# neggles/neurosis

Hardware: AMD Instinct MI355X
Metric: train images/sec (node) SDXL 1024^2 (higher is better)
Workload: dtype bf16

## Files before the change

include/neurosis_hip.h:

```cpp
#ifndef NEUROSIS_HIP_H
#define NEUROSIS_HIP_H

#ifdef __cplusplus
extern "C" {
#endif

const char* nk_last_error(void);
int nk_abi_version(void);

int nk_linear_fwd(const void* x, const void* w, const float* bias, const void* residual, void* y,
                  int M, int N, int K, long ldx, long ldw, long ldr, long ldy, float alpha, void* stream);
int nk_linear_dgrad(const void* dy, const void* w, const void* dx_add, void* dx, int M, int N, int K,
                    long lddy, long ldw, long ldadd, long lddx, void* stream);
long nk_linear_fwd_geglu_ok(int M, int I, int K);
int nk_linear_fwd_geglu(const void* x, const void* w, const float* bias, void* u, void* h, int M, int I, int K, long ldx, long ldw, long ldu,
                        long ldh, void* stream);
int nk_linear_dgrad_geglu(const void* dy, const void* w, const void* u, void* du, int M, int N, int I, long lddy, long ldw, long ldu,
                          long lddu, void* stream);
int nk_linear_fwd_geglu_s(const void* x, const void* w, const float* bias, void* s, void* h, int M, int I, int K, long ldx, long ldw, long lds,
                          long ldh, void* stream);
int nk_linear_dgrad_geglu_s(const void* dy, const void* w, const void* s, void* du, int M, int N, int I, long lddy, long ldw, long lds,
                            long lddu, void* stream);
int nk_linear_wgrad(const void* dy, const void* x, float* dw, int M, int N, int K, long lddy, long ldx,
                    long lddw, int accumulate, void* stream);
int nk_linear_wgrad_bias(const void* dy, const void* x, float* dw, float* dbias, int M, int N, int K, long lddy, long ldx, long lddw,
                         int accumulate, void* stream);

int nk_gemm_sk_status(void);

int nk_health_status(void);
int nk_health_clear(void);
int nk_health_export(int* dst, void* stream);
int nk_health_import(const int* src, void* stream);
int nk_debug_raise_health(void* stream);
int nk_debug_stamp(unsigned long long* dst, void* stream);
int nk_debug_launch_log(int mode);
long nk_debug_launch_names(char* buf, long cap);

int nk_colsum_batched(const void* dy, float* out, float* ws, long M, int N, long ld, int nbatch, int accumulate, void* stream);

int nk_linear_fwd_batched(const void* const* x, const void* const* w, void* const* y, int count, int M, int N, int K,
                          long ldx, long ldw, long ldy, void* stream);

int nk_linear_wgrad_batched(const void* const* dy, const void* const* x, float* const* dw, float* const* dbias, int count, int M, int N,
                            int K, long lddy, long ldx, long lddw, int accumulate, void* stream);

typedef struct NkConvDesc {
  int N, H, W, Cin;
  int Cout, KH, KW;
  int stride;
  int pad_t, pad_l;
  int Ho, Wo;
  int upsample;
} NkConvDesc;
int nk_conv2d_fwd(const NkConvDesc* d, const void* x, const void* w, const float* bias, const void* rowvec,
                  const void* residual, void* y, void* stream);
long nk_conv2d_stats_tiles(const NkConvDesc* d, int stats_groups);
int nk_conv2d_fwd_stats(const NkConvDesc* d, const void* x, const void* w, const float* bias, const void* rowvec, const void* residual,
                        void* y, float* stats_part, int stats_groups, void* stream);
int nk_conv3x3_few_channels_fwd(const void* x, const void* w, const float* bias, void* y, int N, int H, int W, int Cout, int cin_real,
                                void* stream);
int nk_conv_weight_flip(const void* w, void* wt, int Cout, int Cin, int taps, void* stream);
long nk_conv2d_dgrad_flipped_ok(const NkConvDesc* d);
int nk_conv2d_dgrad_flipped(const NkConvDesc* d, const void* dy, const void* wt, void* dx, void* stream);
int nk_conv2d_dgrad(const NkConvDesc* d, const void* dy, const void* w, void* dx, void* stream);
int nk_conv2d_wgrad(const NkConvDesc* d, const void* dy, const void* x, float* dw, int accumulate, void* stream);
int nk_conv2d_wgrad_bias(const NkConvDesc* d, const void* dy, const void* x, float* dw, float* dbias, int accumulate, void* stream);

typedef struct NkAttnDesc {
  int B, H, Lq, Lk, D;
  long sq, sk, sv, so;
  long bq, bk, bv, bo;
  long sdq, sdk, sdv, sdo;
  long bdq, bdk, bdv, bdo;
  float scale;
  int causal;
} NkAttnDesc;
int nk_attention_fwd(const NkAttnDesc* d, const void* q, const void* k, const void* v, void* o, float* lse,
                     void* stream);
long nk_attention_bwd_ws_floats(const NkAttnDesc* d);
int nk_attention_bwd(const NkAttnDesc* d, const void* q, const void* k, const void* v, const void* o,
                     const float* lse, const void* d_o, void* dq, void* dk, void* dv, float* delta_ws, void* stream);
int nk_attention_bwd_causal(const NkAttnDesc* d, const void* q, const void* k, const void* v, const void* o,
                            const float* lse, const void* d_o, void* dq, void* dk, void* dv, void* stream);
int nk_attention_relbias_fwd(const NkAttnDesc* d, const void* q, const void* k, const void* v, void* o, const float* rel, void* stream);
int nk_attention_relbias_fwd_lse(const NkAttnDesc* d, const void* q, const void* k, const void* v, void* o, float* lse, const float* rel, void* stream);
long nk_attention_relbias_bwd_ws_floats(const NkAttnDesc* d);
int nk_attention_relbias_bwd(const NkAttnDesc* d, const void* q, const void* k, const void* v, const void* o, const float* lse, const void* d_o, void* dq,
                             void* dk, void* dv, const float* rel, float* d_rel, float* ws, int accumulate, void* stream);
int nk_relbias_bucket_sum(const float* d_rel, const int* buckets, float* d_weight, int H, int L, int num_buckets, int accumulate, void* stream);
int nk_softmax_rows(void* s, long M, int L, void* stream);

long nk_groupnorm_ws_floats(int N, int HW, int C, int G);
int nk_groupnorm_fwd(const void* x, const float* gamma, const float* beta, void* y, float* mean, float* rstd,
                     float* ws, int N, int HW, int C, int G, float eps, int silu, void* stream);
int nk_groupnorm_sums(const void* x, float* sums, float* ws, int N, int HW, int C, int G, void* stream);
long nk_groupnorm_sums_ws_floats(int N, int nparts, int G);
int nk_groupnorm_sums_from_parts(const float* part, float* sums, float* ws, int N, int nparts, int G, void* stream);
int nk_groupnorm_apply(const void* x, const float* sums, const float* gamma, const float* beta, void* y, float* mean, float* rstd,
                       int N, int HW, int C, int G, float eps, int silu, void* stream);
int nk_groupnorm_bwd(const void* dy, const void* x, const float* gamma, const float* beta, const float* mean,
                     const float* rstd, const void* dx_add, void* dx, float* dgamma, float* dbeta, float* ws,
                     int N, int HW, int C, int G, int silu, int accumulate, void* stream);
int nk_groupnorm_mod_fwd(const void* x, const float* gamma, const float* beta, const void* mod, void* y, float* mean, float* rstd,
                         float* ws, int N, int HW, int C, int G, float eps, int silu, void* stream);
int nk_groupnorm_mod_apply(const void* x, const float* sums, const float* gamma, const float* beta, const void* mod, void* y, float* mean,
                           float* rstd, int N, int HW, int C, int G, float eps, int silu, void* stream);
int nk_groupnorm_mod_bwd(const void* dy, const void* x, const float* gamma, const float* beta, const void* mod, const float* mean,
                         const float* rstd, const void* dx_add, void* dx, float* dgamma, float* dbeta, void* dmod, float* ws,
                         int N, int HW, int C, int G, int silu, int accumulate, void* stream);

int nk_layernorm_fwd(const void* x, const float* gamma, const float* beta, void* y, float* mean, float* rstd,
                     int M, int C, float eps, void* stream);
long nk_layernorm_ws_floats(int M, int C);
int nk_rmsnorm_fwd(const void* x, const float* gamma, void* y, int M, int C, float eps, void* stream);
int nk_rmsnorm_fwd_rstd(const void* x, const float* gamma, void* y, float* rstd, int M, int C, float eps, void* stream);
long nk_rmsnorm_bwd_ws_floats(int M, int C);
int nk_rmsnorm_bwd(const void* dy, const void* x, const float* gamma, const float* rstd, const void* dx_add, void* dx, float* dgamma, float* ws, int M, int C,
                   int accumulate, void* stream);
int nk_layernorm_bwd(const void* dy, const void* x, const float* gamma, const float* mean, const float* rstd,
// ... 189 lines not shown
```

neurosis_amd/csrc/elementwise.hip:

```cpp
#include "../../include/neurosis_hip.h"
#include "nk_common.h"
#include "nk_ew.h"
#include "nk_reduce.h"
#include "norm_plan.h"

struct GegluFwd {
  const bf16_t* u; bf16_t* y; int I;
  __device__ void operator()(long, long row, int ch) const {
    float a[8], g[8];
    ew_load(u + row * 2 * I + ch * 8, a);
    ew_load(u + row * 2 * I + I + ch * 8, g);
#pragma unroll
    for (int e = 0; e < 8; ++e) a[e] *= gelu_erf(g[e]);
    ew_store(y + row * I + ch * 8, a);
  }
};
struct GegluBwd {
  const bf16_t *dy, *u; bf16_t* du; int I;
  __device__ void operator()(long, long row, int ch) const {
    float a[8], g[8], d[8], da[8], dg[8];
    ew_load(u + row * 2 * I + ch * 8, a);
    ew_load(u + row * 2 * I + I + ch * 8, g);
    ew_load(dy + row * I + ch * 8, d);
#pragma unroll
// ... 415 lines not shown
    if (p < HW && c < Cpad) dst[((long)n * HW + p) * Cpad + c] = f2bf(tile[tx][j]);
  }
}
template <typename DstT>
__global__ void nhwc_to_nchw_kernel(const bf16_t* __restrict__ src, DstT* __restrict__ dst, int C, int HW, int Cpad) {
  __shared__ float tile[32][33];
  const int n = blockIdx.z;
  const int p0 = blockIdx.x * 32, c0 = blockIdx.y * 32;
  const int tx = threadIdx.x & 31, ty = threadIdx.x >> 5;
  for (int j = ty; j < 32; j += 8) {
    int p = p0 + j, c = c0 + tx;
    tile[j][tx] = (p < HW && c < C) ? bf2f(src[((long)n * HW + p) * Cpad + c]) : 0.f;
  }
  __syncthreads();
  for (int j = ty; j < 32; j += 8) {
    int c = c0 + j, p = p0 + tx;
    if (c < C && p < HW) {
      float v = tile[tx][j];
      if constexpr (sizeof(DstT) == 4) dst[((long)n * C + c) * HW + p] = v;
      else dst[((long)n * C + c) * HW + p] = f2bf(v);
    }
  }
}
__global__ __launch_bounds__(256) void conv_weight_flip_kernel(const bf16_t* __restrict__ w, bf16_t* __restrict__ wt, int Cout, int Cin, int taps) {
  __shared__ bf16_t tile[64][64 + 8];
  const int tap = blockIdx.z, co0 = blockIdx.y * 64, ci0 = blockIdx.x * 64;
  const int tid = threadIdx.x;
#pragma unroll
  for (int it = 0; it < 2; ++it) {
    const int idx = tid + 256 * it;
    const int r = idx >> 3, ch = idx & 7;
    uint4_t v = {0u, 0u, 0u, 0u};
    if (co0 + r < Cout && ci0 + ch * 8 < Cin) v = *(const uint4_t*)(w + ((long)(co0 + r) * taps + tap) * Cin + ci0 + ch * 8);
    const bf16_t* e = (const bf16_t*)&v;
#pragma unroll
    for (int k = 0; k < 8; ++k) tile[ch * 8 + k][r] = e[k];
  }
  __syncthreads();
  const int tflip = taps - 1 - tap;
#pragma unroll
  for (int it = 0; it < 2; ++it) {
    const int idx = tid + 256 * it;
    const int r = idx >> 3, ch = idx & 7;
    if (ci0 + r < Cin && co0 + ch * 8 < Cout)
      *(uint4_t*)(wt + ((long)(ci0 + r) * taps + tflip) * Cout + co0 + ch * 8) = *(const uint4_t*)&tile[r][ch * 8];
  }
}
extern "C" int nk_conv_weight_flip(const void* w, void* wt, int Cout, int Cin, int taps, void* stream) {
  NK_CHECK_ARG(w && wt && Cout > 0 && Cin > 0 && taps > 0 && taps <= 65535);
  NK_CHECK_ARG((Cout & 7) == 0 && (Cin & 7) == 0);
  hipLaunchKernelGGL(conv_weight_flip_kernel, dim3((Cin + 63) / 64, (Cout + 63) / 64, taps), dim3(256), 0, (hipStream_t)stream, (const bf16_t*)w, (bf16_t*)wt,
                     Cout, Cin, taps);
  return nk_check_launch("conv_weight_flip_kernel");
}

__global__ __launch_bounds__(256) void conv3x3_few_channels_kernel(const bf16_t* __restrict__ x, const bf16_t* __restrict__ w, const float* __restrict__ bias,
                                                                   bf16_t* __restrict__ y, int N, int H, int W, int Cout, int groups_per_wave) {
  const int lane = threadIdx.x & 63, wave = threadIdx.x >> 6;
  const int r = lane & 15, g = lane >> 4;
  const int co_base = blockIdx.y * 128;
  bf16x8_t wf[8][2];
#pragma unroll
  for (int b = 0; b < 8; ++b) {
    const int co = co_base + b * 16 + r;
    uint2_t t0 = {0u, 0u}, t1 = {0u, 0u}, t8 = {0u, 0u};
    if (co < Cout) {
      t0 = *(const uint2_t*)(w + ((long)co * 9 + 2 * g) * 8);
      t1 = *(const uint2_t*)(w + ((long)co * 9 + 2 * g + 1) * 8);
      if (g == 0) t8 = *(const uint2_t*)(w + ((long)co * 9 + 8) * 8);
    }
    wf[b][0] = __builtin_bit_cast(bf16x8_t, (uint4_t){t0.x, t0.y, t1.x, t1.y});
    wf[b][1] = __builtin_bit_cast(bf16x8_t, (uint4_t){t8.x, t8.y, 0u, 0u});
  }
  const int nloc = (g & 1) * 16 + (g >> 1) * 8;
  float bv[4][8];
#pragma unroll
  for (int h = 0; h < 4; ++h)
#pragma unroll
    for (int e = 0; e < 8; ++e) {
      const int co = co_base + h * 32 + nloc + e;
      bv[h][e] = (bias && co < Cout) ? bias[co] : 0.f;
    }
  const long total = (long)N * H * W;
  const long gw = (long)blockIdx.x * 4 + wave;
  const int HW = H * W;
  const int ta = 2 * g, tb = 2 * g + 1;
  const int dya = ta / 3 - 1, dxa = ta % 3 - 1, dyb = tb / 3 - 1, dxb = tb % 3 - 1;

  auto fetch = [&](long grp, uint2_t& a, uint2_t& b, uint2_t& c) {
    a = (uint2_t){0u, 0u}; b = a; c = a;
    const long pix = grp * 16 + r;
    if (pix >= total) return;
    const int n = (int)(pix / HW);
    const int rem = (int)(pix - (long)n * HW);
    const int py = rem / W, px = rem - py * W;
    const bf16_t* img = x + (long)n * HW * 8;
    int yy = py + dya, xx = px + dxa;
    if ((unsigned)yy < (unsigned)H && (unsigned)xx < (unsigned)W) a = *(const uint2_t*)(img + ((long)yy * W + xx) * 8);
    yy = py + dyb; xx = px + dxb;
    if ((unsigned)yy < (unsigned)H && (unsigned)xx < (unsigned)W) b = *(const uint2_t*)(img + ((long)yy * W + xx) * 8);
    if (g == 0) {
      yy = py + 1; xx = px + 1;
      if (yy < H && xx < W) c = *(const uint2_t*)(img + ((long)yy * W + xx) * 8);
    }
  };

// ... 470 lines not shown
```

neurosis_amd/csrc/ops_gemm.hip:

```cpp
#include "../../include/neurosis_hip.h"
#include "nk_gemm.h"
#include <string.h>

static NkGemmParams zero_params() {
  NkGemmParams p;
  memset(&p, 0, sizeof(p));
  p.alpha = 1.0f;
  p.fRowsPerBatch = make_fastdiv(1);
  p.ga.fWo = p.ga.fHoWo = p.ga.fC = p.ga.fKW = make_fastdiv(1);
  p.gb.fWo = p.gb.fHoWo = p.gb.fC = p.gb.fKW = make_fastdiv(1);
  p.tw.fCout = make_fastdiv(1);
  return p;
}

extern "C" int nk_linear_fwd(const void* x, const void* w, const float* bias, const void* residual, void* y,
                             int M, int N, int K, long ldx, long ldw, long ldr, long ldy, float alpha,
                             void* stream) {
  NkGemmParams p = zero_params();
  p.A = (const bf16_t*)x; p.lda = ldx;
  p.B = (const bf16_t*)w; p.ldb = ldw;
  p.M = M; p.N = N; p.K = K;
  p.C = y; p.ldc = ldy;
  p.bias = bias;
  p.residual = (const bf16_t*)residual; p.ldr = ldr;
// ... 208 lines not shown
  g.div = d->stride; g.need_even = d->stride - 1;
  g.fWo = make_fastdiv(Win); g.fHoWo = make_fastdiv(Hin * Win);
  g.fC = make_fastdiv(d->Cout); g.fKW = make_fastdiv(d->KW);
  p.A = (const bf16_t*)dy; p.ga = g;
  p.B = (const bf16_t*)w;
  p.tw.co_stride = (long)d->KH * d->KW * d->Cin;
  p.tw.tap_stride = d->Cin;
  p.tw.fCout = make_fastdiv(d->Cout);
  p.M = d->N * Hin * Win; p.N = d->Cin; p.K = d->KH * d->KW * d->Cout;
  p.C = dx; p.ldc = d->Cin;
  return nk_gemm_dispatch(p, NK_OP_KCG, NK_OP_MCT, 0, 0, (hipStream_t)stream);
}

extern "C" long nk_conv2d_dgrad_flipped_ok(const NkConvDesc* d) {
  if (check_conv(d) || d->KH != 3 || d->KW != 3 || d->stride != 1 || d->pad_t != 1 || d->pad_l != 1) return 0;
  const int Hin = d->upsample ? 2 * d->H : d->H, Win = d->upsample ? 2 * d->W : d->W;
  if (d->Ho != Hin || d->Wo != Win) return 0;
  NkConvDesc t = *d;
  t.H = Hin; t.W = Win; t.Cin = d->Cout; t.Cout = d->Cin; t.upsample = 0;
  NkGemmParams p = conv_fwd_params(&t, nullptr, nullptr, nullptr, nullptr, nullptr, nullptr);
  return nk_halo_tiles_per_image(p, nullptr) > 0;
}

extern "C" int nk_conv2d_dgrad_flipped(const NkConvDesc* d, const void* dy, const void* wt, void* dx, void* stream) {
  NK_CHECK_ARG(nk_conv2d_dgrad_flipped_ok(d) == 1);
  const int Hin = d->upsample ? 2 * d->H : d->H, Win = d->upsample ? 2 * d->W : d->W;
  NkConvDesc t = *d;
  t.H = Hin; t.W = Win; t.Cin = d->Cout; t.Cout = d->Cin; t.upsample = 0;
  NkGemmParams p = conv_fwd_params(&t, dy, wt, nullptr, nullptr, nullptr, dx);
  return nk_gemm_dispatch(p, NK_OP_KCG, NK_OP_KC, 0, 0, (hipStream_t)stream);
}

static int conv_wgrad(const NkConvDesc* d, const void* dy, const void* x, float* dw, float* dbias, int accumulate, void* stream) {
  if (int e = check_conv(d)) return e;
  NkGemmParams p = zero_params();
  p.A = (const bf16_t*)dy; p.lda = d->Cout;
  p.B = (const bf16_t*)x; p.gb = fwd_gather(d);
  p.M = d->Cout; p.N = d->KH * d->KW * d->Cin; p.K = d->N * d->Ho * d->Wo;
  p.C = dw; p.ldc = p.N;
  p.accumulate = accumulate;
  p.dbias = dbias;
  p.halo_nb = (d->KH == 3 && d->KW == 3) ? d->N : 0;
  return nk_gemm_dispatch(p, NK_OP_MC, NK_OP_MCG, 1, 1, (hipStream_t)stream);
}
extern "C" int nk_conv2d_wgrad(const NkConvDesc* d, const void* dy, const void* x, float* dw, int accumulate,
                               void* stream) {
  return conv_wgrad(d, dy, x, dw, nullptr, accumulate, stream);
}
extern "C" int nk_conv2d_wgrad_bias(const NkConvDesc* d, const void* dy, const void* x, float* dw, float* dbias, int accumulate,
                                    void* stream) {
  NK_CHECK_ARG(dbias != nullptr);
  return conv_wgrad(d, dy, x, dw, dbias, accumulate, stream);
}
```

neurosis_amd/lib.py:

```python
from __future__ import annotations

import ctypes as C
import os
from pathlib import Path

import torch

CSRC = Path(__file__).resolve().parent / "csrc"
LIB_PATH = CSRC / "libneurosis_hip.so"

vp, i32, i64, f32 = C.c_void_p, C.c_int, C.c_long, C.c_float


class NkConvDesc(C.Structure):
    _fields_ = [(n, i32) for n in ("N", "H", "W", "Cin", "Cout", "KH", "KW", "stride", "pad_t", "pad_l", "Ho", "Wo", "upsample")]


class NkAttnDesc(C.Structure):
    _fields_ = (
        [(n, i32) for n in ("B", "H", "Lq", "Lk", "D")]
        + [(n, i64) for n in ("sq", "sk", "sv", "so", "bq", "bk", "bv", "bo", "sdq", "sdk", "sdv", "sdo", "bdq", "bdk", "bdv", "bdo")]
        + [("scale", f32), ("causal", i32)]
    )


NK_COLPART_MAX = 32


class NkColpartBatch(C.Structure):
    _fields_ = [("part", vp * NK_COLPART_MAX), ("dgamma", vp * NK_COLPART_MAX), ("dbeta", vp * NK_COLPART_MAX), ("nrows", i32 * NK_COLPART_MAX),
                ("C", i32 * NK_COLPART_MAX), ("accumulate", i32 * NK_COLPART_MAX), ("n", i32)]


cdp, adp = C.POINTER(NkConvDesc), C.POINTER(NkAttnDesc)

SIGNATURES: dict[str, list] = {
    "nk_linear_fwd": [vp, vp, vp, vp, vp, i32, i32, i32, i64, i64, i64, i64, f32, vp],
    "nk_linear_dgrad": [vp, vp, vp, vp, i32, i32, i32, i64, i64, i64, i64, vp],
    "nk_linear_dgrad_geglu": [vp, vp, vp, vp, i32, i32, i32, i64, i64, i64, i64, vp],
    "nk_linear_fwd_geglu": [vp, vp, vp, vp, vp, i32, i32, i32, i64, i64, i64, i64, vp],
    "nk_linear_fwd_geglu_s": [vp, vp, vp, vp, vp, i32, i32, i32, i64, i64, i64, i64, vp],
    "nk_linear_dgrad_geglu_s": [vp, vp, vp, vp, i32, i32, i32, i64, i64, i64, i64, vp],
    "nk_linear_wgrad": [vp, vp, vp, i32, i32, i32, i64, i64, i64, i32, vp],
    "nk_linear_fwd_batched": [C.POINTER(vp), C.POINTER(vp), C.POINTER(vp), i32, i32, i32, i32, i64, i64, i64, vp],
    "nk_linear_wgrad_batched": [C.POINTER(vp), C.POINTER(vp), C.POINTER(vp), C.POINTER(vp), i32, i32, i32, i32, i64, i64, i64, i32, vp],
    "nk_linear_wgrad_bias": [vp, vp, vp, vp, i32, i32, i32, i64, i64, i64, i32, vp],
    "nk_conv2d_wgrad_bias": [cdp, vp, vp, vp, vp, i32, vp],
    "nk_conv2d_fwd": [cdp, vp, vp, vp, vp, vp, vp, vp],
    "nk_conv2d_fwd_stats": [cdp, vp, vp, vp, vp, vp, vp, vp, i32, vp],
    "nk_conv_weight_flip": [vp, vp, i32, i32, i32, vp],
    "nk_conv3x3_few_channels_fwd": [vp, vp, vp, vp, i32, i32, i32, i32, i32, vp],
    "nk_conv2d_dgrad": [cdp, vp, vp, vp, vp],
    "nk_conv2d_dgrad_flipped": [cdp, vp, vp, vp, vp],
    "nk_conv2d_wgrad": [cdp, vp, vp, vp, i32, vp],
    "nk_attention_fwd": [adp, vp, vp, vp, vp, vp, vp],
    "nk_attention_bwd": [adp, vp, vp, vp, vp, vp, vp, vp, vp, vp, vp, vp],
    "nk_attention_bwd_causal": [adp, vp, vp, vp, vp, vp, vp, vp, vp, vp, vp],
    "nk_attention_relbias_fwd": [adp, vp, vp, vp, vp, vp, vp],
    "nk_attention_relbias_fwd_lse": [adp, vp, vp, vp, vp, vp, vp, vp],
    "nk_attention_relbias_bwd": [adp, vp, vp, vp, vp, vp, vp, vp, vp, vp, vp, vp, vp, i32, vp],
    "nk_relbias_bucket_sum": [vp, vp, vp, i32, i32, i32, i32, vp],
    "nk_softmax_rows": [vp, i64, i32, vp],
    "nk_softmax_rows_bwd": [vp, vp, i64, i32, f32, vp],
    "nk_groupnorm_fwd": [vp, vp, vp, vp, vp, vp, vp, i32, i32, i32, i32, f32, i32, vp],
    "nk_groupnorm_sums": [vp, vp, vp, i32, i32, i32, i32, vp],
    "nk_groupnorm_sums_from_parts": [vp, vp, vp, i32, i32, i32, vp],
    "nk_groupnorm_apply": [vp, vp, vp, vp, vp, vp, vp, i32, i32, i32, i32, f32, i32, vp],
    "nk_groupnorm_bwd": [vp, vp, vp, vp, vp, vp, vp, vp, vp, vp, vp, i32, i32, i32, i32, i32, i32, vp],
    "nk_groupnorm_mod_fwd": [vp, vp, vp, vp, vp, vp, vp, vp, i32, i32, i32, i32, f32, i32, vp],
    "nk_groupnorm_mod_apply": [vp, vp, vp, vp, vp, vp, vp, vp, i32, i32, i32, i32, f32, i32, vp],
    "nk_groupnorm_mod_bwd": [vp, vp, vp, vp, vp, vp, vp, vp, vp, vp, vp, vp, vp, i32, i32, i32, i32, i32, i32, vp],
    "nk_layernorm_fwd": [vp, vp, vp, vp, vp, vp, i32, i32, f32, vp],
    "nk_rmsnorm_fwd": [vp, vp, vp, i32, i32, f32, vp],
    "nk_rmsnorm_fwd_rstd": [vp, vp, vp, vp, i32, i32, f32, vp],
    "nk_rmsnorm_bwd": [vp, vp, vp, vp, vp, vp, vp, vp, i32, i32, i32, vp],
    "nk_layernorm_bwd": [vp, vp, vp, vp, vp, vp, vp, vp, vp, vp, i32, i32, i32, vp],
    "nk_layernorm_bwd_dx": [vp, vp, vp, vp, vp, vp, vp, i32, i32, vp],
    "nk_layernorm_bwd_rows": [vp, vp, vp, vp, vp, vp, vp, vp, i32, i32, vp],
    "nk_colpart_reduce_batch": [C.POINTER(NkColpartBatch), vp],
    "nk_layernorm_bwd_params": [vp, vp, vp, vp, vp, vp, vp, i32, i32, i32, vp],
    "nk_geglu_fwd": [vp, vp, i64, i32, vp],
    "nk_geglu_bwd": [vp, vp, vp, i64, i32, vp],
    "nk_geglu_fwd_s": [vp, vp, vp, i64, i32, vp],
    "nk_geglu_bwd_s": [vp, vp, vp, i64, i32, vp],
    "nk_silu_fwd": [vp, vp, i64, vp],
    "nk_gelu_fwd": [vp, vp, i64, i32, vp],
    "nk_gated_gelu_tanh_fwd": [vp, vp, i64, i32, vp],
    "nk_gelu_bwd": [vp, vp, vp, i64, i32, vp],
    "nk_act_bwd": [vp, vp, vp, i64, i32, vp],
    "nk_gated_gelu_tanh_bwd": [vp, vp, vp, i64, i32, vp],
    "nk_embedding_bwd": [vp, vp, i64, vp, vp, i32, i32, i32, i32, i32, i32, vp],
    "nk_gather_rows_bwd": [vp, i64, vp, vp, i32, i32, i32, vp],
    "nk_wgrad_few_rows": [vp, i64, vp, i64, vp, i64, i32, i32, i32, i32, vp],
    "nk_vq_search": [vp, i64, vp, vp, vp, i64, i32, i32, vp],
    "nk_vq_code_stats": [vp, vp, i64, vp, vp, i64, i32, i32, vp],
    "nk_vq_quantize": [vp, vp, vp, i64, vp, vp, vp, i64, i32, i32, i32, vp],
    "nk_gumbel_logits": [vp, i64, vp, vp, vp, i64, i64, i32, i32, vp],
    "nk_gumbel_noise": [vp, i64, i32, vp, i32, vp],
    "nk_gumbel_softmax_fwd": [vp, i64, vp, vp, i32, f32, vp, vp, vp, vp, i64, i32, vp],
    "nk_gumbel_softmax_bwd": [vp, i64, vp, vp, f32, f32, i64, i32, vp],
    "nk_resample_planes": [vp, vp, vp, vp, vp, vp, i32, vp, vp, vp, i32, i64, i32, i32, i32, i32, vp],
    "nk_vit_patchify": [vp, vp, vp, i32, i32, i32, i32, vp],
    "nk_vit_patchify_bwd": [vp, vp, vp, vp, i32, i32, i32, i32, i32, vp],
    "nk_vit_tokens": [vp, vp, vp, vp, i32, i32, i32, vp],
    "nk_vit_tokens_bwd": [vp, vp, i32, i32, i32, vp],
    "nk_vit_add_ln": [vp, vp, vp, vp, vp, i32, vp, vp, vp, i32, i32, f32, vp],
    "nk_vit_cls_head_fwd": [vp, i64, vp, vp, vp, vp, vp, vp, vp, i32, i32, i32, f32, vp],
# ... 4 lines not shown
    "nk_leaky_relu_bwd": [vp, vp, vp, i64, f32, vp],
    "nk_maxpool2x2_fwd": [vp, vp, i32, i32, i32, i32, vp],
    "nk_maxpool2x2_bwd": [vp, vp, vp, i32, i32, i32, i32, vp],
    "nk_maxpool_fwd": [vp, vp, i32, i32, i32, i32, i32, i32, vp],
    "nk_maxpool_bwd": [vp, vp, vp, i32, i32, i32, i32, i32, i32, vp],
    "nk_lpips_layer_fwd": [vp, vp, vp, vp, vp, i32, i32, i32, f32, i32, vp],
    "nk_lpips_layer_bwd": [vp, vp, vp, vp, vp, i32, i32, i32, f32, vp],
    "nk_batchnorm_fwd": [vp, vp, vp, vp, vp, vp, vp, vp, vp, i64, i32, f32, f32, f32, vp],
    "nk_batchnorm_bwd": [vp, vp, vp, vp, vp, vp, vp, vp, vp, vp, i64, i32, f32, i32, vp],
    "nk_batchnorm_eval": [vp, vp, vp, vp, vp, vp, vp, i64, i32, f32, f32, vp],
    "nk_silu_bwd": [vp, vp, vp, i64, vp],
    "nk_add": [vp, vp, vp, i64, vp],
    "nk_dropout": [vp, vp, vp, i64, i32, i64, i64, i64, vp, i32, i32, f32, vp],
    "nk_dropout_draw": [vp, vp, vp],
    "nk_cat_channels": [vp, vp, vp, i64, i32, i32, vp],
    "nk_split_channels": [vp, vp, vp, i64, i32, i32, vp],
    "nk_upsample2x_bwd": [vp, vp, i32, i32, i32, i32, vp],
    "nk_upsample2x_fwd": [vp, vp, i32, i32, i32, i32, vp],
    "nk_avgpool2x_fwd": [vp, vp, i32, i32, i32, i32, vp],
    "nk_avgpool2x_bwd": [vp, vp, i32, i32, i32, i32, vp],
    "nk_nchw_to_nhwc": [vp, i32, vp, i32, i32, i32, i32, f32, vp],
    "nk_nhwc_to_nchw": [vp, vp, i32, i32, i32, i32, i32, vp],
    "nk_cast_f32_to_bf16": [vp, vp, i64, vp],
    "nk_cast_bf16_to_f32": [vp, vp, i64, vp],
    "nk_colsum": [vp, vp, vp, i64, i32, i64, i32, vp],
    "nk_colsum_batched": [vp, vp, vp, i64, i32, i64, i32, i32, vp],
    "nk_timestep_embedding": [vp, vp, i32, i32, f32, vp],
    "nk_edm_prepare": [vp, vp, vp, vp, vp, vp, i32, i32, i32, i32, vp],
    "nk_edm_prepare_cat": [vp, vp, vp, vp, vp, vp, vp, i32, i32, i32, i32, i32, vp],
    "nk_edm_loss": [vp, vp, vp, vp, vp, vp, vp, vp, i32, i32, i32, i32, f32, vp],
    "nk_sample_prepare": [vp, vp, vp, i32, i32, i32, i32, i32, vp],
    "nk_sample_prepare_cat": [vp, vp, vp, vp, vp, i32, i32, i32, i32, i32, i32, vp],
    "nk_sample_denoise": [vp, vp, vp, vp, f32, vp, i32, i32, i32, i32, i32, vp],
    "nk_sample_euler_step": [vp, vp, vp, vp, vp, vp, f32, vp, vp, i32, i32, i32, i32, i32, vp],
    "nk_adamw_flat": [vp, vp, vp, vp, vp, i64, f32, f32, f32, f32, f32, i32, f32, vp],
    "nk_ema_flat": [vp, vp, i64, f32, vp],
    "nk_debug_raise_health": [vp],
    "nk_debug_stamp": [vp, vp],
    "nk_debug_launch_log": [i32],
    "nk_health_clear": [],
    "nk_health_export": [vp, vp],
    "nk_health_import": [vp, vp],
    "nk_adafactor_init": [vp, vp],
    "nk_adafactor_chunk": [vp, vp],
    "nk_came_chunk": [vp, vp],
    "nk_adamw8bit_step": [vp, vp],
}

SIZE_QUERIES: dict[str, list] = {
    "nk_groupnorm_ws_floats": [i32, i32, i32, i32],
    "nk_groupnorm_sums_ws_floats": [i32, i32, i32],
    "nk_conv2d_stats_tiles": [cdp, i32],
    "nk_conv2d_dgrad_flipped_ok": [cdp],
    "nk_linear_fwd_geglu_ok": [i32, i32, i32],
    "nk_layernorm_ws_floats": [i32, i32],
    "nk_layernorm_part_rows": [i32],
    "nk_colsum_ws_floats": [i64, i32],
    "nk_batchnorm_ws_floats": [i64, i32],
    "nk_lpips_layer_ws_floats": [i32, i32],
    "nk_attention_bwd_ws_floats": [adp],
    "nk_attention_relbias_bwd_ws_floats": [adp],
    "nk_rmsnorm_bwd_ws_floats": [i32, i32],
    "nk_vq_search_ws_floats": [i64, i32],
    "nk_vq_quantize_ws_floats": [i64],
    "nk_gumbel_softmax_ws_floats": [i64],
    "nk_resample_ws_floats": [i64, i32, i32, i32, i32],
    "nk_adafactor_tensor_bytes": [],
    "nk_came_tensor_bytes": [],
    "nk_adamw8bit_tensor_bytes": [],
    "nk_gemm_sk_status": [],
    "nk_health_status": [],
    "nk_debug_launch_names": [C.c_char_p, i64],
}

_lib = None


class NkError(RuntimeError):
    pass


def load() -> C.CDLL:
    global _lib
    if _lib is not None:
        return _lib
    path = Path(os.environ.get("NEUROSIS_HIP_LIB", LIB_PATH))
    if not path.exists():
        raise NkError(
            f"{path} not found: the HIP extension is not built. Run `python -c 'import __graft_entry__ as g; g.build()'` "
            "(or `make -C neurosis_amd/csrc`). There is no CPU fallback for the product path."
        )
    lib = C.CDLL(str(path))
    lib.nk_last_error.restype = C.c_char_p
    lib.nk_last_error.argtypes = []
    lib.nk_abi_version.restype = i32
    lib.nk_abi_version.argtypes = []
    for name, argtypes in SIGNATURES.items():
        fn = getattr(lib, name)
        fn.argtypes = argtypes
        fn.restype = i32
    for name, argtypes in SIZE_QUERIES.items():
        fn = getattr(lib, name)
        fn.argtypes = argtypes
        fn.restype = i64
    _lib = lib
    return lib
# ... 24 lines not shown
```

neurosis_amd/ops.py:

```python
from __future__ import annotations

import ctypes as C
import math
import os
import threading
import weakref
from dataclasses import dataclass
from typing import Callable, Optional

import torch
from torch import Tensor

from . import lib
from .lib import NkAttnDesc, NkConvDesc, call, query

BF16 = torch.bfloat16


class EngineState:

    _live = weakref.WeakSet()

    def __init__(self, wgrad_stream=None):
        self.grad_accumulate = False
# ... 424 lines not shown
            call("nk_geglu_fwd_s", u.data_ptr(), h.data_ptr(), u.data_ptr(), M, I, _stream())
        else:
            h = geglu_fwd(u)[0]
    return u, h, _linear_bwd(x if x_saved is None else x_saved, weight, bias, True)


def _linear_bwd(x_in, weight: Tensor, bias: Optional[Tensor], need_dx: bool):
    def bwd(dy: Tensor, dx_add: Optional[Tensor] = None, geglu_u: Optional[Tensor] = None, geglu_s: Optional[Tensor] = None):
        entry = "nk_linear_dgrad_geglu"
        if geglu_s is not None:
            if geglu_u is not None:
                raise ValueError("linear bwd: geglu_u and geglu_s are exclusive")
            geglu_u, entry = geglu_s, "nk_linear_dgrad_geglu_s"
        x = x_in() if callable(x_in) else x_in
        queued = _wgrad_queue is not None and _wgrad_queue.takes(weight) and dy.is_contiguous() and x.is_contiguous()
        db = grad_flat(bias) if bias is not None else None
        if queued:
            _wgrad_queue.add(dy, x, g2d(weight), db)
        else:
            on_wgrad_stream(lambda: gemm_tn_f32(dy, x, g2d(weight), wgrad_mode(weight), dbias=db), dy, x, owner=weight)
        if not need_dx:
            return None
        if geglu_u is not None:
            if dx_add is not None:
                raise ValueError("linear bwd: geglu_u and dx_add are exclusive")
            M, N = dy.shape
            K = weight.shape[1]
            _check2d(geglu_u, "geglu_u")
            if geglu_u.shape != (M, 2 * K):
                raise ValueError(f"linear bwd: geglu_u must be [{M}, {2 * K}], got {tuple(geglu_u.shape)}")
            du = torch.empty(M, 2 * K, dtype=BF16, device=dy.device)
            wq = w2d(weight)
            call(entry, dy.data_ptr(), wq.data_ptr(), geglu_u.data_ptr(), du.data_ptr(), M, N, K, dy.stride(0), wq.stride(0),
                 geglu_u.stride(0), du.stride(0), _stream())
            return du
        return gemm_nn(dy, w2d(weight), dx_add)

    return bwd


def _conv_desc(N, H, W, Cin, Cout, KH, KW, stride, pad_t, pad_l, Ho, Wo, upsample) -> NkConvDesc:
    return NkConvDesc(N, H, W, Cin, Cout, KH, KW, stride, pad_t, pad_l, Ho, Wo, int(upsample))


def groupnorm_sums(x: Img, groups: int) -> Tensor:
    if x.sums is not None and x.sums.shape == (x.N, 2 * groups):
        return x.sums
    sums = torch.empty(x.N, 2 * groups, dtype=torch.float32, device=x.t.device)
    ws = _ws(query("nk_groupnorm_ws_floats", x.N, x.H * x.W, x.C, groups), x.t.device)
    call("nk_groupnorm_sums", x.t.data_ptr(), sums.data_ptr(), ws.data_ptr(), x.N, x.H * x.W, x.C, groups, _stream())
    return sums


def conv2d_fwd(x: Img, weight: Tensor, bias: Optional[Tensor], stride: int = 1, padding=1, upsample: bool = False,
               rowvec: Optional[Tensor] = None, residual: Optional[Tensor] = None, need_dx: bool = True,
               asym_pad: bool = False, stats_groups: Optional[int] = None, cin_real: Optional[int] = None):
    Cout, Cin, KH, KW = weight.shape
    if x.C != Cin:
        raise ValueError(f"conv2d: input has {x.C} channels, weight expects {Cin}")
    Hin, Win = (2 * x.H, 2 * x.W) if upsample else (x.H, x.W)
    if asym_pad:
        pad_t = pad_l = 0
        Ho = (Hin + 1 - KH) // stride + 1
        Wo = (Win + 1 - KW) // stride + 1
    else:
        pad_t = pad_l = int(padding)
        Ho = (Hin + 2 * pad_t - KH) // stride + 1
        Wo = (Win + 2 * pad_l - KW) // stride + 1
    d = _conv_desc(x.N, x.H, x.W, Cin, Cout, KH, KW, stride, pad_t, pad_l, Ho, Wo, upsample)
    y = torch.empty(x.N * Ho * Wo, Cout, dtype=BF16, device=x.t.device)
    _check2d(x.t, "x")
    if not x.t.is_contiguous():
        raise ValueError("conv2d: x must be dense channels-last")
    tiles = query("nk_conv2d_stats_tiles", C.byref(d), stats_groups) if stats_groups else 0
    sums_out = None
    if tiles:
        dev = x.t.device
        part = torch.empty(x.N, tiles, 2 * stats_groups, dtype=torch.float32, device=dev)
        call("nk_conv2d_fwd_stats", C.byref(d), x.t.data_ptr(), w2d(weight).data_ptr(), _p(bias), _p(rowvec), _p(residual), y.data_ptr(),
             part.data_ptr(), stats_groups, _stream())
        sums_out = torch.empty(x.N, 2 * stats_groups, dtype=torch.float32, device=dev)
        ws = _ws(query("nk_groupnorm_sums_ws_floats", x.N, tiles, stats_groups), dev)
        call("nk_groupnorm_sums_from_parts", part.data_ptr(), sums_out.data_ptr(), ws.data_ptr(), x.N, tiles, stats_groups, _stream())
    elif (cin_real in (3, 4) and Cin == 8 and KH == 3 and KW == 3 and stride == 1 and pad_t == 1 and not asym_pad and not upsample and rowvec is None
          and residual is None and Cout % 8 == 0):
        call("nk_conv3x3_few_channels_fwd", x.t.data_ptr(), w2d(weight).data_ptr(), _p(bias), y.data_ptr(), x.N, x.H, x.W, Cout, cin_real, _stream())
    else:
        call("nk_conv2d_fwd", C.byref(d), x.t.data_ptr(), w2d(weight).data_ptr(), _p(bias), _p(rowvec), _p(residual), y.data_ptr(), _stream())
    out = Img(y, x.N, Ho, Wo, sums_out)

    def bwd(dy: Tensor):
        _check2d(dy, "dy")
        if not dy.is_contiguous():
            raise ValueError("conv2d bwd: dy must be dense")
        acc = state_of(weight).grad_accumulate

        if weight.requires_grad:
            if bias is not None:
                on_wgrad_stream(lambda: call("nk_conv2d_wgrad_bias", C.byref(d), dy.data_ptr(), x.t.data_ptr(), g2d(weight).data_ptr(), grad_flat(bias).data_ptr(),
                                             wgrad_mode(weight), _stream()), dy, x.t, owner=weight)
            else:
                on_wgrad_stream(lambda: call("nk_conv2d_wgrad", C.byref(d), dy.data_ptr(), x.t.data_ptr(), g2d(weight).data_ptr(), wgrad_mode(weight), _stream()),
                                dy, x.t, owner=weight)
        drow = None
        if rowvec is not None:
            drow32 = torch.empty(x.N, Cout, dtype=torch.float32, device=dy.device)
            ws = _ws(x.N * query("nk_colsum_ws_floats", Ho * Wo, Cout), dy.device)
            call("nk_colsum_batched", dy.data_ptr(), drow32.data_ptr(), ws.data_ptr(), Ho * Wo, Cout, dy.stride(0), x.N, 0, _stream())
            drow = cast_bf16(drow32)
        dx = None
        if need_dx:
            dxt = torch.empty(x.N * Hin * Win, Cin, dtype=BF16, device=dy.device)
            if query("nk_conv2d_dgrad_flipped_ok", C.byref(d)):
                wt = torch.empty(Cin * 9 * Cout, dtype=BF16, device=dy.device)
                call("nk_conv_weight_flip", w2d(weight).data_ptr(), wt.data_ptr(), Cout, Cin, 9, _stream())
                call("nk_conv2d_dgrad_flipped", C.byref(d), dy.data_ptr(), wt.data_ptr(), dxt.data_ptr(), _stream())
            else:
                call("nk_conv2d_dgrad", C.byref(d), dy.data_ptr(), w2d(weight).data_ptr(), dxt.data_ptr(), _stream())
            if upsample:
                dsm = torch.empty(x.N * x.H * x.W, Cin, dtype=BF16, device=dy.device)
                call("nk_upsample2x_bwd", dxt.data_ptr(), dsm.data_ptr(), x.N, x.H, x.W, Cin, _stream())
                dxt = dsm
            dx = Img(dxt, x.N, x.H, x.W)
        return dx, drow

    return out, bwd


def groupnorm_fwd(x: Img, weight: Tensor, bias: Tensor, groups: int, eps: float, silu: bool, mod: Optional[Tensor] = None):
    what = "groupnorm" if mod is None else "groupnorm_mod"
    if not x.t.is_contiguous():
        raise ValueError(f"{what}: x must be dense channels-last")
    N, HW, Cc = x.N, x.H * x.W, x.C
    if mod is not None:
        _check2d(mod, "mod")
        if tuple(mod.shape) != (N, 2 * Cc) or not mod.is_contiguous():
            raise ValueError(f"groupnorm_mod: mod must be a dense [{N}, {2 * Cc}] (scale | shift) matrix, got {tuple(mod.shape)}")
    entry, mp = "nk_" + what, () if mod is None else (mod.data_ptr(),)
    y = torch.empty_like(x.t)
    mean = torch.empty(N, groups, dtype=torch.float32, device=x.t.device)
    rstd = torch.empty_like(mean)
    nws = query("nk_groupnorm_ws_floats", N, HW, Cc, groups)
    if x.sums is not None and x.sums.shape == (N, 2 * groups):
        call(entry + "_apply", x.t.data_ptr(), x.sums.data_ptr(), weight.data_ptr(), bias.data_ptr(), *mp, y.data_ptr(), mean.data_ptr(),
             rstd.data_ptr(), N, HW, Cc, groups, float(eps), int(silu), _stream())
    else:
        ws = _ws(nws, x.t.device)
        call(entry + "_fwd", x.t.data_ptr(), weight.data_ptr(), bias.data_ptr(), *mp, y.data_ptr(), mean.data_ptr(), rstd.data_ptr(),
             ws.data_ptr(), N, HW, Cc, groups, float(eps), int(silu), _stream())

    def bwd(dy: Tensor, dx_add: Optional[Tensor] = None):
        dx = torch.empty_like(x.t)
        dmod = () if mod is None else (torch.empty_like(mod),)
        ws2 = _ws(nws, dy.device)
        call(entry + "_bwd", dy.data_ptr(), x.t.data_ptr(), weight.data_ptr(), bias.data_ptr(), *mp, mean.data_ptr(), rstd.data_ptr(),
             _p(dx_add), dx.data_ptr(), grad_flat(weight).data_ptr(), grad_flat(bias).data_ptr(), *(t.data_ptr() for t in dmod), ws2.data_ptr(),
             N, HW, Cc, groups, int(silu), int(state_of(weight).grad_accumulate), _stream())
        return (dx, *dmod) if dmod else dx

    return Img(y, x.N, x.H, x.W), bwd


def groupnorm_mod_fwd(x: Img, weight: Tensor, bias: Tensor, mod: Tensor, groups: int, eps: float, silu: bool):
    if mod is None:
# ... 1064 lines not shown
```

Measured before the change: 26.79.

## Decompose upsample-2x 3x3 convs into four 2x2 phase convolutions

Nearest-upsample followed by a 3x3 conv is rewritten as four sub-pixel phase convolutions with pre-summed 2x2 kernels evaluated on the low-resolution input, then pixel-shuffled. Backward uses a single stride-2 4x4 conv for dgrad and per-phase wgrads folded back into 3x3 weights. This cuts the MAC count for the upsample convs by more than half and skips the separate upsample backward pass. In exchange it adds phase-weight preparation, shuffle/unshuffle passes, extra workspace, and bf16 rounding of the summed weights.

```diff
diff --git a/include/neurosis_hip.h b/include/neurosis_hip.h
--- a/include/neurosis_hip.h
+++ b/include/neurosis_hip.h
@@ -66,6 +66,16 @@
 int nk_conv2d_dgrad(const NkConvDesc* d, const void* dy, const void* w, void* dx, void* stream);
 int nk_conv2d_wgrad(const NkConvDesc* d, const void* dy, const void* x, float* dw, int accumulate, void* stream);
 int nk_conv2d_wgrad_bias(const NkConvDesc* d, const void* dy, const void* x, float* dw, float* dbias, int accumulate, void* stream);
+
+int nk_up2_phase_weights(const void* w, void* wp, void* wd, int Cout, int Cin, void* stream);
+long nk_conv2d_up2_ws_bytes(const NkConvDesc* d, int direction);
+int nk_conv2d_up2_fwd(const NkConvDesc* d, const void* x, const void* wp, const float* bias, void* y, void* ws, void* stream);
+int nk_conv2d_up2_dgrad(const NkConvDesc* d, const void* dy, const void* wd, void* dx, void* stream);
+int nk_conv2d_up2_wgrad(const NkConvDesc* d, const void* dy, const void* x, float* dw, int accumulate, void* ws, void* stream);
+int nk_conv2d_up2_wgrad_bias(const NkConvDesc* d, const void* dy, const void* x, float* dw, float* dbias, int accumulate, void* ws, void* stream);
+int nk_pixel_shuffle2x(const void* phases, void* y, int N, int H, int W, int C, void* stream);
+int nk_pixel_unshuffle2x(const void* y, void* phases, int N, int H, int W, int C, void* stream);
+int nk_up2_fold_wgrad(const float* dwp, const float* dbias_p, float* dw, float* dbias, int Cout, int Cin, int accumulate, void* stream);
 
 typedef struct NkAttnDesc {
   int B, H, Lq, Lk, D;
diff --git a/neurosis_amd/csrc/elementwise.hip b/neurosis_amd/csrc/elementwise.hip
--- a/neurosis_amd/csrc/elementwise.hip
+++ b/neurosis_amd/csrc/elementwise.hip
@@ -491,6 +491,113 @@
   hipLaunchKernelGGL(conv_weight_flip_kernel, dim3((Cin + 63) / 64, (Cout + 63) / 64, taps), dim3(256), 0, (hipStream_t)stream, (const bf16_t*)w, (bf16_t*)wt,
                      Cout, Cin, taps);
   return nk_check_launch("conv_weight_flip_kernel");
+}
+
+__global__ __launch_bounds__(256) void up2_phase_weights_kernel(const bf16_t* __restrict__ w, bf16_t* __restrict__ wp, bf16_t* __restrict__ wd, int Cout,
+                                                                int Cin) {
+  __shared__ bf16_t tile[64][64 + 8];
+  const int z = blockIdx.z, co0 = blockIdx.y * 64, ci0 = blockIdx.x * 64;
+  const int a = z >> 3, b = (z >> 2) & 1, u = (z >> 1) & 1, v = z & 1;
+  const int kh0 = u ? 1 + a : 0, khn = 1 + (u ^ a), kw0 = v ? 1 + b : 0, kwn = 1 + (v ^ b);
+  const int tid = threadIdx.x;
+#pragma unroll
+  for (int it = 0; it < 2; ++it) {
+    const int idx = tid + 256 * it;
+    const int r = idx >> 3, ch = idx & 7;
+    float acc[8] = {0.f, 0.f, 0.f, 0.f, 0.f, 0.f, 0.f, 0.f};
+    const bool in = co0 + r < Cout && ci0 + ch * 8 < Cin;
+    if (in) {
+      for (int kh = kh0; kh < kh0 + khn; ++kh)
+        for (int kw = kw0; kw < kw0 + kwn; ++kw) {
+          float f[8];
+          ew_load(w + ((long)(co0 + r) * 9 + kh * 3 + kw) * Cin + ci0 + ch * 8, f);
+#pragma unroll
+          for (int k = 0; k < 8; ++k) acc[k] += f[k];
+        }
+    }
+    const uint4_t o = pack8(acc);
+    if (in) *(uint4_t*)(wp + (((long)(z >> 2) * Cout + co0 + r) * 4 + (z & 3)) * Cin + ci0 + ch * 8) = o;
+    const bf16_t* e = (const bf16_t*)&o;
+#pragma unroll
+    for (int k = 0; k < 8; ++k) tile[ch * 8 + k][r] = e[k];
+  }
+  if (!wd) return;
+  __syncthreads();
+  const int tap = (2 * (1 - u) + (1 - a)) * 4 + 2 * (1 - v) + (1 - b);
+#pragma unroll
+  for (int it = 0; it < 2; ++it) {
+    const int idx = tid + 256 * it;
+    const int r = idx >> 3, ch = idx & 7;
+    if (ci0 + r < Cin && co0 + ch * 8 < Cout)
+      *(uint4_t*)(wd + ((long)(ci0 + r) * 16 + tap) * Cout + co0 + ch * 8) = *(const uint4_t*)&tile[r][ch * 8];
+  }
+}
+extern "C" int nk_up2_phase_weights(const void* w, void* wp, void* wd, int Cout, int Cin, void* stream) {
+  NK_CHECK_ARG(w && wp && Cout > 0 && Cin > 0 && (Cout & 7) == 0 && (Cin & 7) == 0 && (Cout + 63) / 64 <= 65535);
+  NK_CHECK_ARG(nk_aligned16(w) && nk_aligned16(wp) && nk_aligned16(wd));
+  hipLaunchKernelGGL(up2_phase_weights_kernel, dim3((Cin + 63) / 64, (Cout + 63) / 64, 16), dim3(256), 0, (hipStream_t)stream, (const bf16_t*)w,
+                     (bf16_t*)wp, (bf16_t*)wd, Cout, Cin);
+  return nk_check_launch("up2_phase_weights_kernel");
+}
+
+struct PixelShuffle2x {
+  const bf16_t* ph; bf16_t* y; int N, H, W, C;
+  __device__ void operator()(long i, int n, int h, int w, int ch) const {
+    const int p = (h & 1) * 2 + (w & 1);
+    *(uint4_t*)(y + i * 8) = *(const uint4_t*)(ph + ((((long)p * N + n) * H + (h >> 1)) * W + (w >> 1)) * C + ch * 8);
+  }
+};
+struct PixelUnshuffle2x {
+  const bf16_t* y; bf16_t* ph; int N, H, W, C;
+  __device__ void operator()(long i, int pn, int h, int w, int ch) const {
+    const int p = pn / N, n = pn - p * N;
+    *(uint4_t*)(ph + i * 8) = *(const uint4_t*)(y + (((long)n * 2 * H + 2 * h + (p >> 1)) * 2 * W + 2 * w + (p & 1)) * C + ch * 8);
+  }
+};
+extern "C" int nk_pixel_shuffle2x(const void* phases, void* y, int N, int H, int W, int C, void* stream) {
+  NK_CHECK_ARG(phases && y && N > 0 && H > 0 && W > 0 && C > 0 && (C & 7) == 0 && nk_aligned16(phases) && nk_aligned16(y));
+  NK_CHECK_ARG(4l * N < (1l << 31) && 2l * H < (1l << 31) && 2l * W < (1l << 31));
+  return nk_ew_pixels("pixel_shuffle2x", stream, N, 2 * H, 2 * W, C >> 3, PixelShuffle2x{(const bf16_t*)phases, (bf16_t*)y, N, H, W, C});
+}
+extern "C" int nk_pixel_unshuffle2x(const void* y, void* phases, int N, int H, int W, int C, void* stream) {
+  NK_CHECK_ARG(phases && y && N > 0 && H > 0 && W > 0 && C > 0 && (C & 7) == 0 && nk_aligned16(phases) && nk_aligned16(y));
+  NK_CHECK_ARG(4l * N < (1l << 31) && 2l * H < (1l << 31) && 2l * W < (1l << 31));
+  return nk_ew_pixels("pixel_unshuffle2x", stream, 4 * N, H, W, C >> 3, PixelUnshuffle2x{(const bf16_t*)y, (bf16_t*)phases, N, H, W, C});
+}
+
+struct Up2FoldWgrad {
+  const float* dwp; const float* dbp; float* dw; float* dbias; int Cout, Cin, add; long nw;
+  __device__ void operator()(long i) const {
+    float4_t s = {0.f, 0.f, 0.f, 0.f};
+    float* dst;
+    if (i < nw) {
+      const int c4 = Cin >> 2;
+      const long row = i / c4;
+      const int ci = (int)(i - row * c4) * 4;
+      const long co = row / 9;
+      const int tap = (int)(row - co * 9), kh = tap / 3, kw = tap - kh * 3;
+#pragma unroll
+      for (int p = 0; p < 4; ++p) {
+        const int uv = (kh > (p >> 1)) * 2 + (kw > (p & 1));
+        s += *(const float4_t*)(dwp + (((long)p * Cout + co) * 4 + uv) * Cin + ci);
+      }
+      dst = dw + row * Cin + ci;
+    } else {
+      const long co = (i - nw) * 4;
+#pragma unroll
+      for (int p = 0; p < 4; ++p) s += *(const float4_t*)(dbp + (long)p * Cout + co);
+      dst = dbias + co;
+    }
+    if (add) s += *(const float4_t*)dst;
+    *(float4_t*)dst = s;
+  }
+};
+extern "C" int nk_up2_fold_wgrad(const float* dwp, const float* dbias_p, float* dw, float* dbias, int Cout, int Cin, int accumulate, void* stream) {
+  NK_CHECK_ARG(dwp && dw && Cout > 0 && Cin > 0 && (Cout & 7) == 0 && (Cin & 7) == 0 && accumulate >= 0 && accumulate <= 2);
+  NK_CHECK_ARG((dbias == nullptr) == (dbias_p == nullptr));
+  NK_CHECK_ARG(nk_aligned16(dwp) && nk_aligned16(dw) && nk_aligned16(dbias_p) && nk_aligned16(dbias));
+  const long nw = (long)Cout * 9 * (Cin >> 2);
+  return nk_ew_flat("up2_fold_wgrad", stream, nw + (dbias ? Cout >> 2 : 0), Up2FoldWgrad{dwp, dbias_p, dw, dbias, Cout, Cin, accumulate == 1, nw});
 }
 
 __global__ __launch_bounds__(256) void conv3x3_few_channels_kernel(const bf16_t* __restrict__ x, const bf16_t* __restrict__ w, const float* __restrict__ bias,
diff --git a/neurosis_amd/csrc/ops_gemm.hip b/neurosis_amd/csrc/ops_gemm.hip
--- a/neurosis_amd/csrc/ops_gemm.hip
+++ b/neurosis_amd/csrc/ops_gemm.hip
@@ -284,3 +284,76 @@
   NK_CHECK_ARG(dbias != nullptr);
   return conv_wgrad(d, dy, x, dw, dbias, accumulate, stream);
 }
+
+static int check_up2(const NkConvDesc* d) {
+  if (int e = check_conv(d)) return e;
+  NK_CHECK_ARG(d->upsample == 1 && d->KH == 3 && d->KW == 3 && d->stride == 1 && d->pad_t == 1 && d->pad_l == 1);
+  NK_CHECK_ARG(d->Ho == 2 * d->H && d->Wo == 2 * d->W);
+  return NK_OK;
+}
+static NkConvDesc up2_phase_desc(const NkConvDesc* d, int phase) {
+  NkConvDesc t = *d;
+  t.KH = t.KW = 2; t.pad_t = 1 - (phase >> 1); t.pad_l = 1 - (phase & 1);
+  t.Ho = d->H; t.Wo = d->W; t.upsample = 0;
+  return t;
+}
+static size_t up2_align(size_t b) { return (b + 255) & ~(size_t)255; }
+static size_t up2_phase_image_bytes(const NkConvDesc* d) { return up2_align((size_t)4 * d->N * d->H * d->W * d->Cout * sizeof(bf16_t)); }
+static size_t up2_phase_wgrad_bytes(const NkConvDesc* d) { return up2_align((size_t)16 * d->Cout * d->Cin * sizeof(float)); }
+
+extern "C" long nk_conv2d_up2_ws_bytes(const NkConvDesc* d, int direction) {
+  if (check_up2(d) || direction < 0 || direction > 2) return -1;
+  if (direction == 0) return (long)up2_phase_image_bytes(d);
+  if (direction == 1) return 0;
+  return (long)(up2_phase_image_bytes(d) + up2_phase_wgrad_bytes(d) + up2_align((size_t)4 * d->Cout * sizeof(float)));
+}
+
+extern "C" int nk_conv2d_up2_fwd(const NkConvDesc* d, const void* x, const void* wp, const float* bias, void* y, void* ws, void* stream) {
+  if (int e = check_up2(d)) return e;
+  NK_CHECK_ARG(x && wp && y && ws && nk_aligned16(ws));
+  const size_t img = (size_t)d->N * d->H * d->W * d->Cout;
+  for (int ph = 0; ph < 4; ++ph) {
+    const NkConvDesc t = up2_phase_desc(d, ph);
+    NkGemmParams p = conv_fwd_params(&t, x, (const bf16_t*)wp + (size_t)ph * d->Cout * 4 * d->Cin, bias, nullptr, nullptr, (bf16_t*)ws + ph * img);
+    if (int e = nk_gemm_dispatch(p, NK_OP_KCG, NK_OP_KC, 0, 0, (hipStream_t)stream)) return e;
+  }
+  if (nk_launch_log_mode() == 3) return NK_OK;
+  return nk_pixel_shuffle2x(ws, y, d->N, d->H, d->W, d->Cout, stream);
+}
+
+extern "C" int nk_conv2d_up2_dgrad(const NkConvDesc* d, const void* dy, const void* wd, void* dx, void* stream) {
+  if (int e = check_up2(d)) return e;
+  NK_CHECK_ARG(dy && wd && dx);
+  NkConvDesc t = *d;
+  t.H = 2 * d->H; t.W = 2 * d->W; t.Cin = d->Cout; t.Cout = d->Cin;
+  t.KH = t.KW = 4; t.stride = 2; t.Ho = d->H; t.Wo = d->W; t.upsample = 0;
+  if (int e = check_conv(&t)) return e;
+  NkGemmParams p = conv_fwd_params(&t, dy, wd, nullptr, nullptr, nullptr, dx);
+  return nk_gemm_dispatch(p, NK_OP_KCG, NK_OP_KC, 0, 0, (hipStream_t)stream);
+}
+
+static int conv_up2_wgrad(const NkConvDesc* d, const void* dy, const void* x, float* dw, float* dbias, int accumulate, void* ws, void* stream) {
+  if (int e = check_up2(d)) return e;
+  NK_CHECK_ARG(dy && x && dw && ws && nk_aligned16(ws) && accumulate >= 0 && accumulate <= 2);
+  const int plan_only = nk_launch_log_mode() == 3;
+  bf16_t* dyp = (bf16_t*)ws;
+  float* dwp = (float*)((char*)ws + up2_phase_image_bytes(d));
+  float* dbp = dbias ? (float*)((char*)dwp + up2_phase_wgrad_bytes(d)) : nullptr;
+  if (!plan_only)
+    if (int e = nk_pixel_unshuffle2x(dy, dyp, d->N, d->H, d->W, d->Cout, stream)) return e;
+  const size_t img = (size_t)d->N * d->H * d->W * d->Cout;
+  for (int ph = 0; ph < 4; ++ph) {
+    const NkConvDesc t = up2_phase_desc(d, ph);
+    if (int e = conv_wgrad(&t, dyp + ph * img, x, dwp + (size_t)ph * d->Cout * 4 * d->Cin, dbp ? dbp + (size_t)ph * d->Cout : nullptr, 0, stream)) return e;
+  }
+  if (plan_only) return NK_OK;
+  return nk_up2_fold_wgrad(dwp, dbp, dw, dbias, d->Cout, d->Cin, accumulate, stream);
+}
+extern "C" int nk_conv2d_up2_wgrad(const NkConvDesc* d, const void* dy, const void* x, float* dw, int accumulate, void* ws, void* stream) {
+  return conv_up2_wgrad(d, dy, x, dw, nullptr, accumulate, ws, stream);
+}
+extern "C" int nk_conv2d_up2_wgrad_bias(const NkConvDesc* d, const void* dy, const void* x, float* dw, float* dbias, int accumulate, void* ws,
+                                        void* stream) {
+  NK_CHECK_ARG(dbias != nullptr);
+  return conv_up2_wgrad(d, dy, x, dw, dbias, accumulate, ws, stream);
+}
diff --git a/neurosis_amd/lib.py b/neurosis_amd/lib.py
--- a/neurosis_amd/lib.py
+++ b/neurosis_amd/lib.py
@@ -53,6 +53,14 @@
     "nk_conv2d_dgrad": [cdp, vp, vp, vp, vp],
     "nk_conv2d_dgrad_flipped": [cdp, vp, vp, vp, vp],
     "nk_conv2d_wgrad": [cdp, vp, vp, vp, i32, vp],
+    "nk_up2_phase_weights": [vp, vp, vp, i32, i32, vp],
+    "nk_conv2d_up2_fwd": [cdp, vp, vp, vp, vp, vp, vp],
+    "nk_conv2d_up2_dgrad": [cdp, vp, vp, vp, vp],
+    "nk_conv2d_up2_wgrad": [cdp, vp, vp, vp, i32, vp, vp],
+    "nk_conv2d_up2_wgrad_bias": [cdp, vp, vp, vp, vp, i32, vp, vp],
+    "nk_pixel_shuffle2x": [vp, vp, i32, i32, i32, i32, vp],
+    "nk_pixel_unshuffle2x": [vp, vp, i32, i32, i32, i32, vp],
+    "nk_up2_fold_wgrad": [vp, vp, vp, vp, i32, i32, i32, vp],
     "nk_attention_fwd": [adp, vp, vp, vp, vp, vp, vp],
     "nk_attention_bwd": [adp, vp, vp, vp, vp, vp, vp, vp, vp, vp, vp, vp],
     "nk_attention_bwd_causal": [adp, vp, vp, vp, vp, vp, vp, vp, vp, vp, vp],
@@ -163,6 +171,7 @@
     "nk_groupnorm_sums_ws_floats": [i32, i32, i32],
     "nk_conv2d_stats_tiles": [cdp, i32],
     "nk_conv2d_dgrad_flipped_ok": [cdp],
+    "nk_conv2d_up2_ws_bytes": [cdp, i32],
     "nk_linear_fwd_geglu_ok": [i32, i32, i32],
     "nk_layernorm_ws_floats": [i32, i32],
     "nk_layernorm_part_rows": [i32],
diff --git a/neurosis_amd/ops.py b/neurosis_amd/ops.py
--- a/neurosis_amd/ops.py
+++ b/neurosis_amd/ops.py
@@ -500,6 +500,16 @@
     return sums
 
 
+UP2_PHASES_MIN_WORK = 1 << 28
+
+
+def up2_phases_take(pixels: int, Cin: int, Cout: int) -> bool:
+    mode = os.environ.get("NK_UP2_PHASES", "1")
+    if mode == "0":
+        return False
+    return mode == "2" or pixels * Cin * Cout >= UP2_PHASES_MIN_WORK
+
+
 def conv2d_fwd(x: Img, weight: Tensor, bias: Optional[Tensor], stride: int = 1, padding=1, upsample: bool = False,
                rowvec: Optional[Tensor] = None, residual: Optional[Tensor] = None, need_dx: bool = True,
                asym_pad: bool = False, stats_groups: Optional[int] = None, cin_real: Optional[int] = None):
@@ -522,6 +532,8 @@
         raise ValueError("conv2d: x must be dense channels-last")
     tiles = query("nk_conv2d_stats_tiles", C.byref(d), stats_groups) if stats_groups else 0
     sums_out = None
+    up2 = (upsample and KH == 3 and KW == 3 and stride == 1 and pad_t == 1 and not asym_pad and rowvec is None and residual is None and not tiles
+           and up2_phases_take(x.N * x.H * x.W, Cin, Cout))
     if tiles:
         dev = x.t.device
         part = torch.empty(x.N, tiles, 2 * stats_groups, dtype=torch.float32, device=dev)
@@ -533,9 +545,25 @@
     elif (cin_real in (3, 4) and Cin == 8 and KH == 3 and KW == 3 and stride == 1 and pad_t == 1 and not asym_pad and not upsample and rowvec is None
           and residual is None and Cout % 8 == 0):
         call("nk_conv3x3_few_channels_fwd", x.t.data_ptr(), w2d(weight).data_ptr(), _p(bias), y.data_ptr(), x.N, x.H, x.W, Cout, cin_real, _stream())
+    elif up2:
+        dev = x.t.device
+        wp = torch.empty(16 * Cout * Cin, dtype=BF16, device=dev)
+        wd = torch.empty(16 * Cout * Cin, dtype=BF16, device=dev) if need_dx else None
+        call("nk_up2_phase_weights", w2d(weight).data_ptr(), wp.data_ptr(), _p(wd), Cout, Cin, _stream())
+        ws = torch.empty(query("nk_conv2d_up2_ws_bytes", C.byref(d), 0), dtype=torch.uint8, device=dev)
+        call("nk_conv2d_up2_fwd", C.byref(d), x.t.data_ptr(), wp.data_ptr(), _p(bias), y.data_ptr(), ws.data_ptr(), _stream())
+        del wp, ws
     else:
         call("nk_conv2d_fwd", C.byref(d), x.t.data_ptr(), w2d(weight).data_ptr(), _p(bias), _p(rowvec), _p(residual), y.data_ptr(), _stream())
     out = Img(y, x.N, Ho, Wo, sums_out)
+
+    def up2_wgrad(dy: Tensor):
+        ws = torch.empty(query("nk_conv2d_up2_ws_bytes", C.byref(d), 2), dtype=torch.uint8, device=dy.device)
+        if bias is not None:
+            call("nk_conv2d_up2_wgrad_bias", C.byref(d), dy.data_ptr(), x.t.data_ptr(), g2d(weight).data_ptr(), grad_flat(bias).data_ptr(), wgrad_mode(weight),
+                 ws.data_ptr(), _stream())
+        else:
+            call("nk_conv2d_up2_wgrad", C.byref(d), dy.data_ptr(), x.t.data_ptr(), g2d(weight).data_ptr(), wgrad_mode(weight), ws.data_ptr(), _stream())
 
     def bwd(dy: Tensor):
         _check2d(dy, "dy")
@@ -543,7 +571,9 @@
             raise ValueError("conv2d bwd: dy must be dense")
         acc = state_of(weight).grad_accumulate
 
-        if weight.requires_grad:
+        if weight.requires_grad and up2:
+            on_wgrad_stream(lambda: up2_wgrad(dy), dy, x.t, owner=weight)
+        elif weight.requires_grad:
             if bias is not None:
                 on_wgrad_stream(lambda: call("nk_conv2d_wgrad_bias", C.byref(d), dy.data_ptr(), x.t.data_ptr(), g2d(weight).data_ptr(), grad_flat(bias).data_ptr(),
                                              wgrad_mode(weight), _stream()), dy, x.t, owner=weight)
@@ -557,7 +587,11 @@
             call("nk_colsum_batched", dy.data_ptr(), drow32.data_ptr(), ws.data_ptr(), Ho * Wo, Cout, dy.stride(0), x.N, 0, _stream())
             drow = cast_bf16(drow32)
         dx = None
-        if need_dx:
+        if need_dx and up2:
+            dxt = torch.empty(x.N * x.H * x.W, Cin, dtype=BF16, device=dy.device)
+            call("nk_conv2d_up2_dgrad", C.byref(d), dy.data_ptr(), wd.data_ptr(), dxt.data_ptr(), _stream())
+            dx = Img(dxt, x.N, x.H, x.W)
+        elif need_dx:
             dxt = torch.empty(x.N * Hin * Win, Cin, dtype=BF16, device=dy.device)
             if query("nk_conv2d_dgrad_flipped_ok", C.byref(d)):
                 wt = torch.empty(Cin * 9 * Cout, dtype=BF16, device=dy.device)
```

Result: faster. 27.12, median of 6 (+1.2%).
